# cteufel13/VisualOdometry

Hardware: AMD Instinct MI355X
Metric: BA GN-iters/sec at 50 poses×20k landmarks; descriptor-match Mpairs/sec (higher is better)
Workload: dtype f64; 1 GPU; cfg3: synthetic sliding-window BA window, 50 poses x 20000 landmarks, 83108 observations (seed 3, KITTI K, first 2 poses fixed, lambda=1.0); one step = one full GN iteration; poses=50, landmarks=20000, observations=83108, parallelism=landmark-sharded x1, k1_variant=0

## Files before the change

### visualodometry_amd/csrc/ba_lin_wave.h

```cpp
#pragma once

#include <hip/hip_runtime.h>

#include <cstddef>
#include <cstdint>
#include <utility>

#include "ba_kernels.h"
#include "ba_math.h"
#include "vo_common.h"

namespace vo {

namespace {

constexpr double kPivotRelEps = 1e-12;

enum { kPhLoad = 0, kPhBacksub, kPhLinObs, kPhReduce, kPhElim, kPhSchur, kPhWrite, kPhSchurU, kPhT0, kPhT1,
       kPhObs, kPhTe, kPhPts, kPhPairs, kPhSlots, kPhCams, kPhEnd };
static_assert(kPhEnd == kPhCount, "K1 stamp row (ba_kernels.h)");
template <bool kStamp>
struct Stamper {
  unsigned long long t = 0, acc[kPhCount] = {};
  bool lead = false;
  int row = 0;
  __device__ __forceinline__ void start(bool ld, int r) {
    lead = kStamp && ld;
    row = r;
    if (lead) {
      acc[kPhT0] = t = __builtin_amdgcn_s_memtime();
      unsigned xcc;
      asm volatile("s_getreg_b32 %0, hwreg(HW_REG_XCC_ID, 0, 4)" : "=s"(xcc));
      const unsigned simd = __builtin_amdgcn_s_getreg(4 | (4 << 6) | ((2 - 1) << 11));
      acc[kPhCams] = (unsigned long long)xcc << 24 | (unsigned long long)simd << 32;
    }
  }
  __device__ __forceinline__ void start() { start(threadIdx.x == 0, blockIdx.x); }
  __device__ __forceinline__ void mark(int ph) {
    if (lead) {
      const unsigned long long n = __builtin_amdgcn_s_memtime();
      acc[ph] += n - t;
      t = n;
    }
  }
  __device__ __forceinline__ void count(int k, int v) {
    if (lead) acc[k] += (unsigned long long)v;
  }
  __device__ __forceinline__ void flush(unsigned long long* out) {
    if (lead) acc[kPhT1] = __builtin_amdgcn_s_memtime();
    if (lead && out)
      for (int k = 0; k < kPhCount; ++k) out[(long)row * kPhCount + k] = acc[k];
  }
};

__device__ __forceinline__ void lds_sync_wave() { asm volatile("s_waitcnt lgkmcnt(0)" ::: "memory"); }

constexpr int kZbStride = 18;
constexpr int kZbR = 6 * kChunkObs;
constexpr int kZbDc = kZbR + 2 * kChunkObs;
constexpr int kZbPoseO = kZbDc + 6 * kSegCams;
static_assert(kZbPoseO + 12 * kSegAllCams <= kChunkTe * kZbStride, "Zb region aliases");

struct alignas(16) LinWave {
  ChunkImg img;
  int spos[kSegSlots];
  int cpos[kSegCams];
  alignas(16) double Jc[kChunkObs][10];
  alignas(16) double zb[kChunkTe * kZbStride];
  alignas(16) double bt[kChunkTe][6];
  double X[kChunkPts][3];
  double L[kChunkPts][6];
  double h[kChunkPts][3];
  alignas(16) double pose_n[kSegAllCams][12];
  uint8_t valid[kChunkPts];
  uint8_t srow[kSegSlots];
  uint8_t crow[kSegCams];
  double wcost;
};
constexpr int kWaveSegsPerCu = 6;
static_assert(sizeof(LinWave) <= 160 * 1024 / kWaveSegsPerCu, "one-wave K1 LDS image");
static_assert(kWaveMaxChunks <= 8 && kWaveMaxChunks * sizeof(LinWave) <= 160 * 1024 &&
                  kWaveItems * 36 * sizeof(double) <= 2176 * sizeof(double),
              "the chunks of a segment fit one CU; every item's block fits the scratch rows");

__device__ __forceinline__ bool point_block_w(const LinWave& S, double lambda, int p, double (&l)[6],
                                              double (&h)[3]) {
  double v00 = 0, v01 = 0, v02 = 0, v11 = 0, v12 = 0, v22 = 0, g0 = 0, g1 = 0, g2 = 0;
  const int o0 = S.img.pt_obs[p], o1 = S.img.pt_obs[p + 1];
  for (int o = o0; o < o1; ++o) {
#pragma unroll
    for (int k = 0; k < 2; ++k) {
      const double a = S.zb[6 * o + 3 * k], b = S.zb[6 * o + 3 * k + 1], c = S.zb[6 * o + 3 * k + 2];
      const double rk = S.zb[kZbR + 2 * o + k];
      v00 += a * a; v01 += a * b; v02 += a * c;
      v11 += b * b; v12 += b * c; v22 += c * c;
      g0 += a * rk; g1 += b * rk; g2 += c * rk;
    }
  }
  v00 += lambda; v11 += lambda; v22 += lambda;
  const double eps = kPivotRelEps * (v00 + v11 + v22);
  bool ok = v00 > eps;
  const double i00 = rsq_nr(ok ? v00 : 1.0);
  const double l10 = v01 * i00, l20 = v02 * i00;
  const double d1 = v11 - l10 * l10;
  ok = ok && d1 > eps;
  const double i11 = rsq_nr(ok ? d1 : 1.0);
  const double l21 = (v12 - l20 * l10) * i11;
  const double d2 = v22 - l20 * l20 - l21 * l21;
  ok = ok && d2 > eps;
  const double i22 = rsq_nr(ok ? d2 : 1.0);
  l[0] = i00; l[1] = l10; l[2] = i11; l[3] = l20; l[4] = l21; l[5] = i22;
  h[0] = g0 * i00;
  h[1] = (g1 - l10 * h[0]) * i11;
  h[2] = (g2 - l20 * h[0] - l21 * h[1]) * i22;
  return ok;
}

template <bool kJc, bool kBack, bool kRob>
__device__ __forceinline__ void obs_lin_w(LinWave& S, const LinArgs& A, const double* T, int o,
                                          const double* dc, double& cost) {
  const int q = S.img.obs_pt[o];
  const double X0 = S.X[q][0], X1 = S.X[q][1], X2 = S.X[q][2];
  const double x = T[0] * X0 + T[1] * X1 + T[2] * X2 + T[9];
  const double y = T[3] * X0 + T[4] * X1 + T[5] * X2 + T[10];
  const double z = T[6] * X0 + T[7] * X1 + T[8] * X2 + T[11];
  const double iz = rcp_nr(z);
  const float2 m = reinterpret_cast<const float2*>(S.img.uv)[o];
  double r0 = A.fx * x * iz + A.cx - (double)m.x;
  double r1 = A.fy * y * iz + A.cy - (double)m.y;
  double j00 = A.fx * iz, j02 = -A.fx * x * iz * iz;
  double j11 = A.fy * iz, j12 = -A.fy * y * iz * iz;
  if constexpr (kRob) {
    double rho;
    const double s = huber_scale(r0, r1, A.huber, A.huber2, rho);
    if (!kBack) cost += rho;
    r0 *= s; r1 *= s;
    j00 *= s; j02 *= s; j11 *= s; j12 *= s;
  }
  if (kBack && dc) {
    r0 += j00 * dc[0] + j02 * dc[2] + (j02 * y) * dc[3] + (j00 * z - j02 * x) * dc[4] - (j00 * y) * dc[5];
    r1 += j11 * dc[1] + j12 * dc[2] + (j12 * y - j11 * z) * dc[3] - (j12 * x) * dc[4] + (j11 * x) * dc[5];
  }
  if (!kBack && !kRob) cost += r0 * r0 + r1 * r1;
  S.zb[kZbR + 2 * o] = r0;
  S.zb[kZbR + 2 * o + 1] = r1;
  if (kJc) {
    double2* jc = reinterpret_cast<double2*>(S.Jc[o]);
    jc[0] = make_double2(j00, j02);
    jc[1] = make_double2(j02 * y, j00 * z - j02 * x);
    jc[2] = make_double2(-j00 * y, j11);
    jc[3] = make_double2(j12, j12 * y - j11 * z);
    jc[4] = make_double2(-j12 * x, j11 * x);
  }
  double* jp = &S.zb[6 * o];
  jp[0] = j00 * T[0] + j02 * T[6];
  jp[1] = j00 * T[1] + j02 * T[7];
  jp[2] = j00 * T[2] + j02 * T[8];
  jp[3] = j11 * T[3] + j12 * T[6];
  jp[4] = j11 * T[4] + j12 * T[7];
  jp[5] = j11 * T[5] + j12 * T[8];
}

__device__ __forceinline__ void jc_load(const LinWave& S, int o, double (&jj)[12]) {
  const double2* jr = reinterpret_cast<const double2*>(S.Jc[o]);
  const double2 a = jr[0], b = jr[1], c = jr[2], d = jr[3], e = jr[4];
  jj[0] = a.x; jj[1] = 0.0; jj[2] = a.y; jj[3] = b.x; jj[4] = b.y; jj[5] = c.x;
  jj[6] = 0.0; jj[7] = c.y; jj[8] = d.x; jj[9] = d.y; jj[10] = e.x; jj[11] = e.y;
}

template <bool kGroup, class Stamp>
__device__ __forceinline__ void schur_block(LinWave& S, const LinArgs& A, int si, bool live, Stamp& st) {
  double out[36];
#pragma unroll
  for (int e = 0; e < 36; ++e) out[e] = 0.0;
  const int e0 = S.img.slotp[si], n = live ? S.img.apcnt[si] : 0;
  const int dcam = S.img.adcam[si], s = S.img.aslot[si];
  if (n > 0) {
    auto zload = [&](int pr, double2 (&zx)[9], double2 (&zy)[9]) {
      const double2* px = reinterpret_cast<const double2*>(&S.zb[kZbStride * (pr & 255)]);
      const double2* py = reinterpret_cast<const double2*>(&S.zb[kZbStride * (pr >> 8)]);
#pragma unroll
      for (int k = 0; k < 9; ++k) {
        zx[k] = px[k];
        zy[k] = py[k];
      }
    };
    auto accum = [&](const double2 (&zx)[9], const double2 (&zy)[9]) {
      const double* x = reinterpret_cast<const double*>(zx);
      const double* y = reinterpret_cast<const double*>(zy);
#pragma unroll
      for (int i = 0; i < 6; ++i)
#pragma unroll
        for (int j = 0; j < 6; ++j) {
          double v = out[6 * i + j];
          v = __builtin_fma(-x[3 * i], y[3 * j], v);
          v = __builtin_fma(-x[3 * i + 1], y[3 * j + 1], v);
          out[6 * i + j] = __builtin_fma(-x[3 * i + 2], y[3 * j + 2], v);
        }
    };
    auto pid = [&](int j) { return (int)S.img.pairs[e0 + min(j, n - 1)]; };
    double2 zxA[9], zyA[9], zxB[9], zyB[9];
    zload(pid(0), zxA, zyA);
    int pn = pid(1);
    int j = 0;
    for (; j + 2 <= n; j += 2) {
      zload(pn, zxB, zyB);
      pn = pid(j + 2);
      accum(zxA, zyA);
      zload(pn, zxA, zyA);
      pn = pid(j + 3);
      accum(zxB, zyB);
    }
    if (j < n) accum(zxA, zyA);
  }
  st.mark(kPhSchur);
  double ob[6] = {0, 0, 0, 0, 0, 0};
  const int u0 = S.img.auo[si], un = live ? S.img.auo[si + 1] - u0 : 0;
  if (un > 0) {
    auto uacc = [&](const double (&jj)[12]) {
#pragma unroll
      for (int i = 0; i < 6; ++i)
#pragma unroll
        for (int c = 0; c < 6; ++c)
          out[6 * i + c] = __builtin_fma(jj[6 + i], jj[6 + c], __builtin_fma(jj[i], jj[c], out[6 * i + c]));
    };
    auto oid = [&](int i) { return (int)S.img.camol[u0 + min(i, un - 1)]; };
    double jA[12], jB[12];
    jc_load(S, oid(0), jA);
    int on = oid(1);
    int i = 0;
    for (; i + 2 <= un; i += 2) {
      jc_load(S, on, jB);
      on = oid(i + 2);
      uacc(jA);
      jc_load(S, on, jA);
      on = oid(i + 3);
      uacc(jB);
    }
    if (i < un) uacc(jA);
  }
  if (n > 0 && dcam != 0xFF) {
    int xn = S.img.pairs[e0] & 255;
    for (int e = 0; e < n; ++e) {
      const double2* br = reinterpret_cast<const double2*>(S.bt[xn]);
      xn = S.img.pairs[e0 + min(e + 1, n - 1)] & 255;
#pragma unroll
      for (int k = 0; k < 3; ++k) {
        const double2 v = br[k];
        ob[2 * k] += v.x;
        ob[2 * k + 1] += v.y;
      }
    }
  }
  if (!live) {
    st.mark(kPhSchurU);
    return;
  }
  if (dcam != 0xFF) {
    double2* bp = reinterpret_cast<double2*>(&S.X[0][0]) + 3 * si;
#pragma unroll
    for (int k = 0; k < 3; ++k) bp[k] = make_double2(ob[2 * k], ob[2 * k + 1]);
  }
  if (!kGroup && S.img.anp[si] <= 1) {
    double2* w = reinterpret_cast<double2*>(&A.slab[36l * S.spos[s]]);
#pragma unroll
    for (int e = 0; e < 18; ++e) w[e] = make_double2(out[2 * e], out[2 * e + 1]);
  } else {
    lds_sync_wave();
    double2* w = reinterpret_cast<double2*>(&S.Jc[0][0]) + 18 * si;
#pragma unroll
    for (int e = 0; e < 18; ++e) w[e] = make_double2(out[2 * e], out[2 * e + 1]);
  }
  st.mark(kPhSchurU);
}

static_assert(offsetof(LinWave, zb) == offsetof(LinWave, Jc) + sizeof(LinWave::Jc) &&
                  offsetof(LinWave, bt) == offsetof(LinWave, zb) + sizeof(LinWave::zb) &&
                  sizeof(LinWave::Jc) + sizeof(LinWave::zb) + sizeof(LinWave::bt) >= 36 * sizeof(double) * kWaveItems,
              "the copies' scratch (kWaveItems items) fits the Jc | Z | bt region");
template <bool kGroup>
__device__ __forceinline__ void copy_rows(LinWave& S, const LinArgs& A, int si, bool live) {
  const int m = S.img.anp[si];
  if (!live || m <= 1) return;
  const int k = S.img.acopy[si], j0 = si - k;
  const int e0 = 36 * k / m, ne = 36 * (k + 1) / m - e0;
  double* sc = &S.Jc[0][0] + 36 * j0 + e0;
  double acc[18];
#pragma unroll
  for (int i = 0; i < 18; ++i) acc[i] = sc[min(i, ne - 1)];
  int c = 1;
  for (; c + 2 <= m; c += 2) {
    double v[18], u[18];
#pragma unroll
    for (int i = 0; i < 18; ++i) {
      v[i] = sc[36 * c + min(i, ne - 1)];
      u[i] = sc[36 * (c + 1) + min(i, ne - 1)];
    }
#pragma unroll
    for (int i = 0; i < 18; ++i) acc[i] = (acc[i] + v[i]) + u[i];
  }
  if (c < m)
#pragma unroll
    for (int i = 0; i < 18; ++i) acc[i] += sc[36 * c + min(i, ne - 1)];
  double* row = kGroup ? sc : &A.slab[36l * S.spos[S.img.aslot[si]] + e0];
#pragma unroll
  for (int i = 0; i < 18; ++i)
    if (i < ne) row[i] = acc[i];
}

template <bool kGroup>
__device__ __forceinline__ void rhs_rows(LinWave& S, const LinArgs& A, int nac, int tid) {
  static_assert(sizeof(S.X) + sizeof(S.L) + sizeof(S.h) >= 6 * sizeof(double) * kWaveSlots &&
                    offsetof(LinWave, L) == offsetof(LinWave, X) + sizeof(S.X) &&
                    offsetof(LinWave, h) == offsetof(LinWave, L) + sizeof(S.L),
                "b partials of every item fit the X | L | h region");
  const double* bp = &S.X[0][0];
  for (int q = tid; q < 6 * nac; q += kLinLanesWave) {
    const int ci = q / 6, a = q - 6 * ci;
    const int j0 = S.img.cdiag0[ci], nj = S.img.cdiagn[ci];
    double acc = 0.0;
    for (int j = 0; j < nj; j += 8) {
      double v[8];
#pragma unroll
      for (int k = 0; k < 8; ++k) v[k] = bp[6 * (j0 + min(j + k, nj - 1)) + a];
#pragma unroll
      for (int k = 0; k < 8; ++k)
        if (j + k < nj) acc += v[k];
    }
    if (kGroup) (&S.pose_n[0][0])[6 * S.img.acid[ci] + a] = acc;
    else A.slab_b[6l * S.cpos[S.img.acid[ci]] + a] = acc;
  }
}

static_assert(sizeof(LinWave::pose_n) >= kSegCams * 6 * sizeof(double), "the chunk's b sums fit pose_n");

__device__ __forceinline__ void slab_store(double2* p, double2 v) {
  typedef double f64x2 __attribute__((ext_vector_type(2)));
  const f64x2 d = {v.x, v.y};
  asm volatile("global_store_dwordx4 %0, %1, off sc1\n\ts_nop 0" ::"v"(p), "v"(d) : "memory");
}

typedef __attribute__((address_space(3))) int lin_lds_int;
struct LinGate {
  const unsigned* pub = nullptr;
  unsigned want = 0;
  int* status = nullptr;
  int iter_tag = 0;
  int timeout_flag = 0;
  lin_lds_int* s_gate = nullptr;
  unsigned long long* stamps = nullptr;
};
constexpr unsigned kLinGateSpins = 1u << 25;

typedef __attribute__((address_space(1))) unsigned long long lin_gu64;
typedef __attribute__((address_space(1))) unsigned lin_gu32;
__device__ __forceinline__ double ld_sc1_f64(const double* p) {
  return __longlong_as_double((long long)__hip_atomic_load((lin_gu64*)p, __ATOMIC_RELAXED, __HIP_MEMORY_SCOPE_AGENT));
}

template <int MODE, bool kStamp, int NW, bool kGated>
__device__ __forceinline__ void lin_wave_body(LinArgs A, LinWave* Sw, int* s_arrive_p, const int seg, const LinGate G) {
  int& s_arrive = *s_arrive_p;
  constexpr bool kGroup = NW > 1;
  constexpr bool kRob = (MODE & kRobust) != 0;
  if constexpr ((MODE & kLm) != 0) A.lambda = *A.lm_lambda;
  constexpr int kCombWaves = NW < 4 ? NW : 4;
  constexpr bool kEarly = NW > kCombWaves && (MODE & kAccum);
  constexpr int kCombS = (kSegSlots * 18 + 64 * kCombWaves - 1) / (64 * kCombWaves);
  constexpr int kCombB = (kSegCams * 3 + 64 * kCombWaves - 1) / (64 * kCombWaves);
  static_assert(kLinLanesWave == 64, "one wave");
  static_assert(!kGated || (MODE & (kBacksub | kAccum | kLm)) == (kBacksub | kAccum), "the gated K1: a GN iteration's");
  const int wv = kGroup ? __builtin_amdgcn_readfirstlane((int)threadIdx.x >> 6) : 0;
  constexpr bool kPrio = kEarly;
  if constexpr (kPrio)
    if (wv >= kCombWaves) __builtin_amdgcn_s_setprio(1);
  auto prio_drop = [&]() __attribute__((always_inline)) {
    if constexpr (kPrio)
      if (wv >= kCombWaves) __builtin_amdgcn_s_setprio(0);
  };
  LinWave& S = Sw[wv];
  const int tid = (int)threadIdx.x & 63, chk = seg * NW + wv;
  Stamper<kStamp> st;
  st.start(tid == 0, chk);
  const int* SH = A.seg_hdr + (long)kSegHdr * seg;
  const int4* SH4 = reinterpret_cast<const int4*>(SH);
  const int16_t* SH16 = reinterpret_cast<const int16_t*>(SH);
  const int stat = !kGated && A.status ? *A.status : 0;
  const int4 g0 = SH4[0], g1 = SH4[1];
  const int4* CH = kGroup ? A.chunk_hdr + 4l * chk : SH4 + 8;
  const int4 h0 = CH[0], h1 = CH[1], h2 = CH[2], h3 = CH[3];
  constexpr int kImgVec = (int)(sizeof(ChunkImg) / 16);
  static_assert(kImgVec > 128 && kImgVec <= 192, "three 16-byte staging granules per lane");
  const uint4* img = reinterpret_cast<const uint4*>(A.chunk_img + chk);
  const uint4 img0 = img[tid], img1 = img[64 + tid], img2 = img[min(128 + tid, kImgVec - 1)];
  int i_acam[3], i_wcam[3];
#pragma unroll
  for (int k = 0; k < 3; ++k) {
    i_acam[k] = SH16[16 + min((tid + 64 * k) / 12, kSegAllCams - 1)];
    i_wcam[k] = SH16[32 + min((tid + 64 * k) / 6, kSegCams - 1)];
  }
  if (kEarly) {
    if (threadIdx.x == 0) s_arrive = 0;
    lds_sync_wave();
    __builtin_amdgcn_s_barrier();
    asm volatile("" ::: "memory");
  }
  if (stat) return;
  const int nslots = g0.x, slot_off = g0.y, cam0 = g0.z, ncams = g0.w, na = g1.x;
  const int nob = h0.y, nte = h0.w, p0 = h1.x, npt = h1.y;
  double* dcw = &S.zb[kZbDc];
  double* pose_o = &S.zb[kZbPoseO];
  double vx[2], vpn[3], vpo[3], vdc[3];
  const long xb = npt > 0 ? 3l * p0 : 0;
#pragma unroll
  for (int k = 0; k < 2; ++k) vx[k] = A.points[xb + min(tid + 64 * k, max(3 * npt - 1, 0))];
#pragma unroll
  for (int k = 0; k < 3; ++k) {
    const int e = tid + 64 * k;
    if (!kGated) vpn[k] = A.pose_new[12l * i_acam[k] + e % 12];
    if (MODE & kBacksub) {
      vpo[k] = A.pose_old[12l * i_acam[k] + e % 12];
      if (!kGated) vdc[k] = A.dc[6l * i_wcam[k] + e % 6];
    }
  }
  int vsp = 0, vcp = 0;
  if ((MODE & kAccum) && nslots > 0) {
    vsp = A.slab_pos[slot_off + min(tid, nslots - 1)];
    vcp = A.cam_pos[cam0 + min(tid, max(ncams - 1, 0))];
  }
  {
    uint4* d = reinterpret_cast<uint4*>(&S.img);
    d[tid] = img0;
    d[64 + tid] = img1;
    if (128 + tid < kImgVec) d[128 + tid] = img2;
  }
#pragma unroll
  for (int k = 0; k < 2; ++k)
    if (tid + 64 * k < 3 * npt) (&S.X[0][0])[tid + 64 * k] = vx[k];
#pragma unroll
  for (int k = 0; k < 3; ++k) {
    const int e = tid + 64 * k;
    if (e < 12 * na) {
      if (!kGated) (&S.pose_n[0][0])[e] = vpn[k];
      if (MODE & kBacksub) pose_o[e] = vpo[k];
    }
    if (!kGated && (MODE & kBacksub) && e < 6 * ncams) dcw[e] = vdc[k];
  }
  if (MODE & kAccum) {
    if (tid < nslots) S.spos[tid] = vsp;
    if (tid < ncams) S.cpos[tid] = vcp;
    if (kGroup) {
      S.srow[tid] = 0xFF;
      if (tid < kSegCams) S.crow[tid] = 0;
    }
  }
  if constexpr (kGated) {
#if VO_BA_STAMPS
    if (G.stamps && threadIdx.x == 0) {
      asm volatile("s_waitcnt vmcnt(0) lgkmcnt(0)" ::: "memory");
      G.stamps[1] = __builtin_amdgcn_s_memrealtime();
    }
#endif
    if (threadIdx.x == 0) {
      unsigned spins = 0, v;
      while (((v = __hip_atomic_load((lin_gu32*)G.pub, __ATOMIC_RELAXED, __HIP_MEMORY_SCOPE_AGENT)) | 1u) !=
             (G.want | 1u)) {
        __builtin_amdgcn_s_sleep(2);
        if (++spins > kLinGateSpins) break;
      }
      int verdict = (int)(v & 1u);
      if ((v | 1u) != (G.want | 1u)) {
        verdict = 1;
        const unsigned prior = __hip_atomic_load((lin_gu32*)G.status, __ATOMIC_RELAXED, __HIP_MEMORY_SCOPE_AGENT);
        __hip_atomic_fetch_or((lin_gu32*)G.status, (unsigned)G.timeout_flag | (prior ? 0u : (unsigned)G.iter_tag),
                              __ATOMIC_RELAXED, __HIP_MEMORY_SCOPE_AGENT);
      }
      *G.s_gate = verdict;
    }
    lds_sync_wave();
    __builtin_amdgcn_s_barrier();
    asm volatile("" ::: "memory");
    if (__builtin_amdgcn_readfirstlane(*(volatile lin_lds_int*)G.s_gate)) return;
#if VO_BA_STAMPS
    if (G.stamps && threadIdx.x == 0) G.stamps[2] = __builtin_amdgcn_s_memrealtime();
#endif
#pragma unroll
    for (int k = 0; k < 3; ++k) {
      const int e = tid + 64 * k;
      vpn[k] = ld_sc1_f64(A.pose_new + 12l * i_acam[k] + e % 12);
      vdc[k] = ld_sc1_f64(A.dc + 6l * i_wcam[k] + e % 6);
    }
#pragma unroll
    for (int k = 0; k < 3; ++k) {
      const int e = tid + 64 * k;
      if (e < 12 * na) (&S.pose_n[0][0])[e] = vpn[k];
      if (e < 6 * ncams) dcw[e] = vdc[k];
    }
  }
  st.count(kPhSlots, nslots);
  st.count(kPhCams, ncams);
  st.count(kPhObs, nob);
  st.count(kPhTe, nte);
  st.count(kPhPts, npt);
  st.count(kPhPairs, h2.y - h2.x);
  double cost = 0.0;
  lds_sync_wave();
  st.mark(kPhLoad);

  if (MODE & kBacksub) {
    if (tid < nob) {
      const int lc = S.img.obs_lcam[tid];
      obs_lin_w<false, true, kRob>(S, A, &pose_o[12 * S.img.acam[tid]], tid, lc >= 0 ? &dcw[6 * lc] : nullptr, cost);
    }
    lds_sync_wave();
    if (tid < npt) {
      double l[6], h[3];
      if (point_block_w(S, A.lambda, tid, l, h)) {
        const double x2 = -h[2] * l[5];
        const double x1 = (-h[1] - l[4] * x2) * l[2];
        const double x0 = (-h[0] - l[1] * x1 - l[3] * x2) * l[0];
        S.X[tid][0] += x0;
        S.X[tid][1] += x1;
        S.X[tid][2] += x2;
        A.points[3l * (p0 + tid)] = S.X[tid][0];
        A.points[3l * (p0 + tid) + 1] = S.X[tid][1];
        A.points[3l * (p0 + tid) + 2] = S.X[tid][2];
      }
    }
    lds_sync_wave();
    st.mark(kPhBacksub);
  }

  if (tid < nob) obs_lin_w<(MODE & kAccum) != 0, false, kRob>(S, A, S.pose_n[S.img.acam[tid]], tid, nullptr, cost);
  if (MODE & kAccum) {
    lds_sync_wave();
    st.mark(kPhLinObs);
    if (tid < npt) {
      double l[6], h[3];
      const bool ok = point_block_w(S, A.lambda, tid, l, h);
      S.valid[tid] = ok;
#pragma unroll
      for (int e = 0; e < 6; ++e) S.L[tid][e] = l[e];
      S.h[tid][0] = ok ? h[0] : 0.0;
      S.h[tid][1] = ok ? h[1] : 0.0;
      S.h[tid][2] = ok ? h[2] : 0.0;
    }
    lds_sync_wave();
    st.mark(kPhReduce);
    {
      double W[18], g[6];
#pragma unroll
      for (int e = 0; e < 18; ++e) W[e] = 0.0;
#pragma unroll
      for (int e = 0; e < 6; ++e) g[e] = 0.0;
      const int t = min(tid, max(nte - 1, 0));
      const bool live = tid < nte;
      const int oa = S.img.te_obs[t], ob = live ? S.img.te_obs[t + 1] : oa;
      for (int o = oa; o < ob; ++o) {
        double jj[12];
        jc_load(S, o, jj);
#pragma unroll
        for (int k = 0; k < 2; ++k) {
          const double rk = S.zb[kZbR + 2 * o + k];
          const double q0 = S.zb[6 * o + 3 * k], q1 = S.zb[6 * o + 3 * k + 1], q2 = S.zb[6 * o + 3 * k + 2];
#pragma unroll
          for (int a = 0; a < 6; ++a) {
            const double jc = jj[6 * k + a];
            W[3 * a] += jc * q0;
            W[3 * a + 1] += jc * q1;
            W[3 * a + 2] += jc * q2;
            g[a] += jc * rk;
          }
        }
      }
      const int p = S.img.te_pt[t];
      const bool use = live && S.valid[p] && S.img.te_lcam[t] >= 0;
      const double i00 = S.L[p][0], l10 = S.L[p][1], i11 = S.L[p][2];
      const double l20 = S.L[p][3], l21 = S.L[p][4], i22 = S.L[p][5];
      const double hh0 = S.h[p][0], hh1 = S.h[p][1], hh2 = S.h[p][2];
      double bt[6];
#pragma unroll
      for (int a = 0; a < 6; ++a) {
        const double z0 = W[3 * a] * i00;
        const double z1 = (W[3 * a + 1] - l10 * z0) * i11;
        const double z2 = (W[3 * a + 2] - l20 * z0 - l21 * z1) * i22;
        W[3 * a] = use ? z0 : 0.0;
        W[3 * a + 1] = use ? z1 : 0.0;
        W[3 * a + 2] = use ? z2 : 0.0;
        bt[a] = use ? -g[a] + (z0 * hh0 + z1 * hh1 + z2 * hh2) : 0.0;
      }
      if (live && !use)
        for (int o = oa; o < ob; ++o)
#pragma unroll
          for (int e = 0; e < 10; ++e) S.Jc[o][e] = 0.0;
      lds_sync_wave();
      if (live) {
        double2* zr = reinterpret_cast<double2*>(&S.zb[kZbStride * t]);
#pragma unroll
        for (int e = 0; e < 9; ++e) zr[e] = make_double2(W[2 * e], W[2 * e + 1]);
        double2* br = reinterpret_cast<double2*>(S.bt[t]);
#pragma unroll
        for (int e = 0; e < 3; ++e) br[e] = make_double2(bt[2 * e], bt[2 * e + 1]);
      }
    }
    lds_sync_wave();
    st.mark(kPhElim);
    prio_drop();

    {
      const int nas = h3.z;
      for (int j = tid; j - tid < nas; j += kLinLanesWave)
        schur_block<kGroup>(S, A, min(j, nas - 1), j < nas, st);
      lds_sync_wave();
      for (int j = tid; j - tid < nas; j += kLinLanesWave) copy_rows<kGroup>(S, A, min(j, nas - 1), j < nas);
      rhs_rows<kGroup>(S, A, h3.w, tid);
      if (kGroup) {
        if (tid < nas && S.img.acopy[tid] == 0) S.srow[S.img.aslot[tid]] = (uint8_t)tid;
        if (tid < h3.w) S.crow[S.img.acid[tid]] = 1;
      }
    }
    st.mark(kPhWrite);
  }
#pragma unroll
  for (int m = 1; m < 64; m <<= 1) cost += __shfl_xor(cost, m, 64);
  if (!kGroup) {
    if (tid == 0) A.slab_cost[seg] = cost;
  } else {
    if (tid == 0) S.wcost = cost;
    const int t = (int)threadIdx.x;
    const int nps = nslots * 18, npb = ncams * 3;
    double2 accS[kCombS], accB[kCombB];
    bool anyS[kCombS], anyB[kCombB];
    double2 *dstS[kCombS], *dstB[kCombB];
    auto comb = [&](auto w0c, auto w1c) __attribute__((always_inline)) {
      constexpr int W0 = decltype(w0c)::value, W1 = decltype(w1c)::value;
#pragma unroll
      for (int k = 0; k < kCombS; ++k) {
        const int p = min(t + 64 * kCombWaves * k, max(nps - 1, 0));
        const int s = p / 18, i = 2 * (p - 18 * s);
        if constexpr (W0 == 0) {
          accS[k] = make_double2(0.0, 0.0);
          anyS[k] = false;
          dstS[k] = reinterpret_cast<double2*>(A.slab + 36l * S.spos[s] + i);
        }
#pragma unroll
        for (int w = W0; w < W1; ++w) {
          const int r = Sw[w].srow[s];
          const double2 v = *reinterpret_cast<const double2*>(&Sw[w].Jc[0][0] + 36 * (r == 0xFF ? 0 : r) + i);
          accS[k].x = r == 0xFF ? accS[k].x : anyS[k] ? accS[k].x + v.x : v.x;
          accS[k].y = r == 0xFF ? accS[k].y : anyS[k] ? accS[k].y + v.y : v.y;
          anyS[k] = anyS[k] || r != 0xFF;
        }
      }
#pragma unroll
      for (int k = 0; k < kCombB; ++k) {
        const int p = min(t + 64 * kCombWaves * k, max(npb - 1, 0));
        const int c = p / 3, i = 2 * (p - 3 * c);
        if constexpr (W0 == 0) {
          accB[k] = make_double2(0.0, 0.0);
          anyB[k] = false;
          dstB[k] = reinterpret_cast<double2*>(A.slab_b + 6l * S.cpos[c] + i);
        }
#pragma unroll
        for (int w = W0; w < W1; ++w) {
          const bool on = Sw[w].crow[c] != 0;
          const double2 v = *reinterpret_cast<const double2*>(&Sw[w].pose_n[0][0] + 6 * c + i);
          accB[k].x = !on ? accB[k].x : anyB[k] ? accB[k].x + v.x : v.x;
          accB[k].y = !on ? accB[k].y : anyB[k] ? accB[k].y + v.y : v.y;
          anyB[k] = anyB[k] || on;
        }
      }
    };
    using std::integral_constant;
    if constexpr (kEarly) {
      if (wv < kCombWaves) {
        lds_sync_wave();
        if (tid == 0) __hip_atomic_fetch_add(&s_arrive, 1, __ATOMIC_RELAXED, __HIP_MEMORY_SCOPE_WORKGROUP);
        while (__builtin_amdgcn_readfirstlane(
                   __hip_atomic_load(&s_arrive, __ATOMIC_RELAXED, __HIP_MEMORY_SCOPE_WORKGROUP)) < kCombWaves)
          __builtin_amdgcn_s_sleep(4);
        asm volatile("" ::: "memory");
        comb(integral_constant<int, 0>{}, integral_constant<int, kCombWaves>{});
      }
    }
    __syncthreads();
    if ((MODE & kAccum) && wv < kCombWaves) {
      comb(integral_constant<int, kEarly ? kCombWaves : 0>{}, integral_constant<int, NW>{});
#pragma unroll
      for (int k = 0; k < kCombS; ++k)
        if (t + 64 * kCombWaves * k < nps) slab_store(dstS[k], accS[k]);
#pragma unroll
      for (int k = 0; k < kCombB; ++k)
        if (t + 64 * kCombWaves * k < npb) slab_store(dstB[k], accB[k]);
    }
    if (t == 0) {
      double c = 0.0;
#pragma unroll
      for (int w = 0; w < NW; ++w) c += Sw[w].wcost;
      A.slab_cost[seg] = c;
    }
  }
  st.mark(kPhWrite);
  st.flush(A.stamps);
#if VO_BA_STAMPS
  if constexpr (kGated)
    if (G.stamps && threadIdx.x == 0) G.stamps[3] = __builtin_amdgcn_s_memrealtime();
#endif
}

}

}
```

Before: 17510 GN-iters/s.

## Hoist pose-only backsubstitution work ahead of the gated K1 wait

In the gated K1 path, the observation projection, Jacobians, residuals and point-block Cholesky factors that depend only on the old pose are computed before spinning on the publication gate. After the gate opens, only the camera-update correction (dc) terms and the point solve remain. This moves work off the critical path of the cross-kernel dependency. It also delays raising wave priority until after the gate and adds an optional macro to drop priority earlier. The reordered FMA arithmetic may change rounding slightly.

New measurement: 17540 GN-iters/s (median of 6 runs). Within noise of the previous version (+0.2%).

```diff
diff --git a/visualodometry_amd/csrc/ba_lin_wave.h b/visualodometry_amd/csrc/ba_lin_wave.h
--- a/visualodometry_amd/csrc/ba_lin_wave.h
+++ b/visualodometry_amd/csrc/ba_lin_wave.h
@@ -161,6 +161,113 @@
   jp[5] = j11 * T[5] + j12 * T[8];
 }
 
+struct BackObs {
+  double j00, j02, j11, j12, x, y, z, r0, r1;
+};
+
+template <bool kRob>
+__device__ __forceinline__ void backsub_obs_pre(LinWave& S, const LinArgs& A, const double* T, int o, BackObs& B) {
+#pragma clang fp contract(off)
+  const int q = S.img.obs_pt[o];
+  const double X0 = S.X[q][0], X1 = S.X[q][1], X2 = S.X[q][2];
+  const double x = T[9] + __builtin_fma(X2, T[2], __builtin_fma(X0, T[0], X1 * T[1]));
+  const double y = T[10] + (kRob ? __builtin_fma(X2, T[5], __builtin_fma(X0, T[3], X1 * T[4]))
+                                 : __builtin_fma(X2, T[5], __builtin_fma(X1, T[4], X0 * T[3])));
+  const double z = T[11] + __builtin_fma(X2, T[8], __builtin_fma(X0, T[6], X1 * T[7]));
+  const double iz = rcp_nr(z);
+  const float2 m = reinterpret_cast<const float2*>(S.img.uv)[o];
+  double r0 = __builtin_fma(A.fx * x, iz, A.cx) - (double)m.x;
+  double r1 = __builtin_fma(A.fy * y, iz, A.cy) - (double)m.y;
+  double j00 = A.fx * iz, j02 = ((-A.fx * x) * iz) * iz;
+  double j11 = A.fy * iz, j12 = ((-A.fy * y) * iz) * iz;
+  if constexpr (kRob) {
+    double rho;
+    const double s = huber_scale(r0, r1, A.huber, A.huber2, rho);
+    r0 *= s; r1 *= s;
+    j00 *= s; j02 *= s; j11 *= s; j12 *= s;
+  }
+  S.zb[kZbR + 2 * o] = r0;
+  S.zb[kZbR + 2 * o + 1] = r1;
+  double* jp = &S.zb[6 * o];
+  jp[0] = __builtin_fma(j00, T[0], j02 * T[6]);
+  jp[1] = __builtin_fma(j00, T[1], j02 * T[7]);
+  jp[2] = __builtin_fma(j00, T[2], j02 * T[8]);
+  jp[3] = __builtin_fma(j11, T[3], j12 * T[6]);
+  jp[4] = __builtin_fma(j11, T[4], j12 * T[7]);
+  jp[5] = __builtin_fma(j11, T[5], j12 * T[8]);
+  B.j00 = j00; B.j02 = j02; B.j11 = j11; B.j12 = j12;
+  B.x = x; B.y = y; B.z = z; B.r0 = r0; B.r1 = r1;
+}
+
+template <bool kRob>
+__device__ __forceinline__ void backsub_obs_dc(LinWave& S, const BackObs& B, const double* dc, int o) {
+#pragma clang fp contract(off)
+  const double t4 = __builtin_fma(B.j00, B.z, -(B.j02 * B.x));
+  const double t3 = __builtin_fma(B.j12, B.y, -(B.j11 * B.z));
+  double e0 = __builtin_fma(B.j00, dc[0], B.j02 * dc[2]);
+  e0 = __builtin_fma(B.j02 * B.y, dc[3], e0);
+  e0 = __builtin_fma(t4, dc[4], e0);
+  e0 = __builtin_fma(-(B.j00 * B.y), dc[5], e0);
+  double e1 = kRob ? __builtin_fma(B.j12, dc[2], B.j11 * dc[1]) : __builtin_fma(B.j11, dc[1], B.j12 * dc[2]);
+  e1 = __builtin_fma(t3, dc[3], e1);
+  e1 = __builtin_fma(-(B.j12 * B.x), dc[4], e1);
+  e1 = __builtin_fma(B.j11 * B.x, dc[5], e1);
+  S.zb[kZbR + 2 * o] = B.r0 + e0;
+  S.zb[kZbR + 2 * o + 1] = B.r1 + e1;
+}
+
+__device__ __forceinline__ bool backsub_point_pre(const LinWave& S, double lambda, int p, double (&l)[6]) {
+#pragma clang fp contract(off)
+  double v00 = 0, v01 = 0, v02 = 0, v11 = 0, v12 = 0, v22 = 0;
+  const int o0 = S.img.pt_obs[p], o1 = S.img.pt_obs[p + 1];
+  for (int o = o0; o < o1; ++o) {
+#pragma unroll
+    for (int k = 0; k < 2; ++k) {
+      const double a = S.zb[6 * o + 3 * k], b = S.zb[6 * o + 3 * k + 1], c = S.zb[6 * o + 3 * k + 2];
+      v00 = __builtin_fma(a, a, v00); v01 = __builtin_fma(a, b, v01); v02 = __builtin_fma(a, c, v02);
+      v11 = __builtin_fma(b, b, v11); v12 = __builtin_fma(b, c, v12); v22 = __builtin_fma(c, c, v22);
+    }
+  }
+  v00 += lambda; v11 += lambda; v22 += lambda;
+  const double eps = kPivotRelEps * (v00 + v11 + v22);
+  bool ok = v00 > eps;
+  const double i00 = rsq_nr(ok ? v00 : 1.0);
+  const double l10 = v01 * i00, l20 = v02 * i00;
+  const double d1 = __builtin_fma(-l10, l10, v11);
+  ok = ok && d1 > eps;
+  const double i11 = rsq_nr(ok ? d1 : 1.0);
+  const double l21 = __builtin_fma(-l20, l10, v12) * i11;
+  const double d2 = __builtin_fma(-l21, l21, __builtin_fma(-l20, l20, v22));
+  ok = ok && d2 > eps;
+  const double i22 = rsq_nr(ok ? d2 : 1.0);
+  l[0] = i00; l[1] = l10; l[2] = i11; l[3] = l20; l[4] = l21; l[5] = i22;
+  return ok;
+}
+
+__device__ __forceinline__ void backsub_point_dc(const LinWave& S, int p, const double (&l)[6], double (&X)[3]) {
+#pragma clang fp contract(off)
+  double g0 = 0, g1 = 0, g2 = 0;
+  const int o0 = S.img.pt_obs[p], o1 = S.img.pt_obs[p + 1];
+  for (int o = o0; o < o1; ++o) {
+#pragma unroll
+    for (int k = 0; k < 2; ++k) {
+      const double a = S.zb[6 * o + 3 * k], b = S.zb[6 * o + 3 * k + 1], c = S.zb[6 * o + 3 * k + 2];
+      const double rk = S.zb[kZbR + 2 * o + k];
+      g0 = __builtin_fma(a, rk, g0); g1 = __builtin_fma(b, rk, g1); g2 = __builtin_fma(c, rk, g2);
+    }
+  }
+  const double h0 = g0 * l[0];
+  const double h1 = __builtin_fma(-l[1], h0, g1) * l[2];
+  const double nh2 = __builtin_fma(-l[4], h1, __builtin_fma(-l[3], h0, g2)) * -l[5];
+  const double x2 = l[5] * nh2;
+  const double t1 = __builtin_fma(-l[4], x2, -h1);
+  const double x1 = l[2] * t1;
+  const double t0 = __builtin_fma(-l[3], x2, __builtin_fma(-l[1], x1, -h0));
+  X[0] = __builtin_fma(l[0], t0, X[0]);
+  X[1] = __builtin_fma(l[2], t1, X[1]);
+  X[2] = __builtin_fma(l[5], nh2, X[2]);
+}
+
 __device__ __forceinline__ void jc_load(const LinWave& S, int o, double (&jj)[12]) {
   const double2* jr = reinterpret_cast<const double2*>(S.Jc[o]);
   const double2 a = jr[0], b = jr[1], c = jr[2], d = jr[3], e = jr[4];
@@ -351,6 +458,9 @@
   unsigned long long* stamps = nullptr;
 };
 constexpr unsigned kLinGateSpins = 1u << 25;
+#ifndef VO_BA_CHAIN_PRIO_DROP
+#define VO_BA_CHAIN_PRIO_DROP 0
+#endif
 
 typedef __attribute__((address_space(1))) unsigned long long lin_gu64;
 typedef __attribute__((address_space(1))) unsigned lin_gu32;
@@ -372,8 +482,12 @@
   static_assert(!kGated || (MODE & (kBacksub | kAccum | kLm)) == (kBacksub | kAccum), "the gated K1: a GN iteration's");
   const int wv = kGroup ? __builtin_amdgcn_readfirstlane((int)threadIdx.x >> 6) : 0;
   constexpr bool kPrio = kEarly;
-  if constexpr (kPrio)
-    if (wv >= kCombWaves) __builtin_amdgcn_s_setprio(1);
+  auto prio_raise = [&]() __attribute__((always_inline)) {
+    if constexpr (kPrio)
+      if (wv >= kCombWaves) __builtin_amdgcn_s_setprio(1);
+  };
+  if constexpr (!kGated) prio_raise();
+  constexpr bool kDropAtReduce = kGated && VO_BA_CHAIN_PRIO_DROP == 1;
   auto prio_drop = [&]() __attribute__((always_inline)) {
     if constexpr (kPrio)
       if (wv >= kCombWaves) __builtin_amdgcn_s_setprio(0);
@@ -454,7 +568,14 @@
       if (tid < kSegCams) S.crow[tid] = 0;
     }
   }
+  BackObs bo = {};
+  double bl[6] = {};
+  bool bok = false;
   if constexpr (kGated) {
+    lds_sync_wave();
+    if (tid < nob) backsub_obs_pre<kRob>(S, A, &pose_o[12 * S.img.acam[tid]], tid, bo);
+    lds_sync_wave();
+    if (tid < npt) bok = backsub_point_pre(S, A.lambda, tid, bl);
 #if VO_BA_STAMPS
     if (G.stamps && threadIdx.x == 0) {
       asm volatile("s_waitcnt vmcnt(0) lgkmcnt(0)" ::: "memory");
@@ -484,6 +605,7 @@
 #if VO_BA_STAMPS
     if (G.stamps && threadIdx.x == 0) G.stamps[2] = __builtin_amdgcn_s_memrealtime();
 #endif
+    prio_raise();
 #pragma unroll
     for (int k = 0; k < 3; ++k) {
       const int e = tid + 64 * k;
@@ -508,23 +630,41 @@
   st.mark(kPhLoad);
 
   if (MODE & kBacksub) {
-    if (tid < nob) {
-      const int lc = S.img.obs_lcam[tid];
-      obs_lin_w<false, true, kRob>(S, A, &pose_o[12 * S.img.acam[tid]], tid, lc >= 0 ? &dcw[6 * lc] : nullptr, cost);
-    }
-    lds_sync_wave();
-    if (tid < npt) {
-      double l[6], h[3];
-      if (point_block_w(S, A.lambda, tid, l, h)) {
-        const double x2 = -h[2] * l[5];
-        const double x1 = (-h[1] - l[4] * x2) * l[2];
-        const double x0 = (-h[0] - l[1] * x1 - l[3] * x2) * l[0];
-        S.X[tid][0] += x0;
-        S.X[tid][1] += x1;
-        S.X[tid][2] += x2;
-        A.points[3l * (p0 + tid)] = S.X[tid][0];
-        A.points[3l * (p0 + tid) + 1] = S.X[tid][1];
-        A.points[3l * (p0 + tid) + 2] = S.X[tid][2];
+    if constexpr (kGated) {
+      if (tid < nob) {
+        const int lc = S.img.obs_lcam[tid];
+        if (lc >= 0) backsub_obs_dc<kRob>(S, bo, &dcw[6 * lc], tid);
+      }
+      lds_sync_wave();
+      if (tid < npt && bok) {
+        double X[3] = {S.X[tid][0], S.X[tid][1], S.X[tid][2]};
+        backsub_point_dc(S, tid, bl, X);
+        S.X[tid][0] = X[0];
+        S.X[tid][1] = X[1];
+        S.X[tid][2] = X[2];
+        A.points[3l * (p0 + tid)] = X[0];
+        A.points[3l * (p0 + tid) + 1] = X[1];
+        A.points[3l * (p0 + tid) + 2] = X[2];
+      }
+    } else {
+      if (tid < nob) {
+        const int lc = S.img.obs_lcam[tid];
+        obs_lin_w<false, true, kRob>(S, A, &pose_o[12 * S.img.acam[tid]], tid, lc >= 0 ? &dcw[6 * lc] : nullptr, cost);
+      }
+      lds_sync_wave();
+      if (tid < npt) {
+        double l[6], h[3];
+        if (point_block_w(S, A.lambda, tid, l, h)) {
+          const double x2 = -h[2] * l[5];
+          const double x1 = (-h[1] - l[4] * x2) * l[2];
+          const double x0 = (-h[0] - l[1] * x1 - l[3] * x2) * l[0];
+          S.X[tid][0] += x0;
+          S.X[tid][1] += x1;
+          S.X[tid][2] += x2;
+          A.points[3l * (p0 + tid)] = S.X[tid][0];
+          A.points[3l * (p0 + tid) + 1] = S.X[tid][1];
+          A.points[3l * (p0 + tid) + 2] = S.X[tid][2];
+        }
       }
     }
     lds_sync_wave();
@@ -547,6 +687,7 @@
     }
     lds_sync_wave();
     st.mark(kPhReduce);
+    if constexpr (kDropAtReduce) prio_drop();
     {
       double W[18], g[6];
 #pragma unroll
@@ -605,7 +746,7 @@
     }
     lds_sync_wave();
     st.mark(kPhElim);
-    prio_drop();
+    if constexpr (!kDropAtReduce) prio_drop();
 
     {
       const int nas = h3.z;
```
